# BraveGroup/DCD

Measured on AMD Instinct MI355X. Metric: images/sec DGDE train step (bs=8, 384x1280), higher is better.
Workload: dtype f32; 1 GPU; DGDE train bs=8 fp32 on 1xMI355X, synthetic KITTI 384x1280 + random kpts_ann (DGDE.yaml, DLA-34+DCNv2, 6 objects/image); global_batch=8, per_gpu_batch=8, input=384x1280, parallelism=dp1, dcn_precision=f32, step_launch=eager, sync_bn=False

## Files before the change

### dcd_amd/csrc/dcn_v2.hip

```cpp

#include <hip/hip_runtime.h>
#include <stdint.h>
#include <stdlib.h>
#include <string.h>
#include <atomic>
#include <map>
#include <vector>
#include <mutex>
#include <utility>

#include "../../include/dcd_hip.h"
#include "tuning_env.h"
#include "lds_limit.h"

typedef float f32x16 __attribute__((ext_vector_type(16)));
typedef float f32x32 __attribute__((ext_vector_type(32)));

namespace {

template <int N> struct IntC {
    static constexpr int value = N;
};

struct Geom {
    int B, C, H, W, Co, kh, kw, sh, sw, ph, pw, dh, dw, dg;
    int Ho, Wo, HoWo, KK, cpg, cpgp, Kp, Cop;
};

__host__ inline int round_up(int x, int m) { return (x + m - 1) / m * m; }

__host__ inline bool make_geom(Geom &g, int B, int C, int H, int W, int Co, int kh, int kw, int sh, int sw, int ph,
                               int pw, int dh, int dw, int dg)
{
    if (B <= 0 || C <= 0 || H <= 0 || W <= 0 || Co <= 0 || kh <= 0 || kw <= 0 || sh <= 0 || sw <= 0 || ph < 0 ||
        pw < 0 || dh <= 0 || dw <= 0 || dg <= 0 || C % dg)
        return false;
    g.B = B; g.C = C; g.H = H; g.W = W; g.Co = Co; g.kh = kh; g.kw = kw; g.sh = sh; g.sw = sw;
    g.ph = ph; g.pw = pw; g.dh = dh; g.dw = dw; g.dg = dg;
    g.Ho = (H + 2 * ph - (dh * (kh - 1) + 1)) / sh + 1;
    g.Wo = (W + 2 * pw - (dw * (kw - 1) + 1)) / sw + 1;
    if (g.Ho <= 0 || g.Wo <= 0) return false;
    g.HoWo = g.Ho * g.Wo;
    g.KK = kh * kw;
    g.cpg = C / dg;
    g.cpgp = round_up(g.cpg, 32);
    g.Kp = dg * g.KK * g.cpgp;
    g.Cop = round_up(Co, 32);
    if ((int64_t)C * H * W >= (1ll << 31) || (int64_t)Co * g.HoWo >= (1ll << 31) ||
        (int64_t)g.Kp * g.Cop >= (1ll << 31) || (int64_t)dg * 2 * g.KK * g.HoWo >= (1ll << 31))
        return false;
    return true;
}

__device__ __forceinline__ void prep_weights_body(const float *__restrict__ w, float *__restrict__ wf, float *__restrict__ wb, const Geom &g,
                                                  int bid, int nb)
{
    const int n = g.Kp * g.Cop;
    for (int idx = bid * blockDim.x + threadIdx.x; idx < n; idx += nb * blockDim.x) {
        const int o = idx / g.Kp, kp = idx - o * g.Kp;
        const int seg = kp / g.cpgp, cc = kp - seg * g.cpgp;
        const int grp = seg / g.KK, t = seg - grp * g.KK;
        float v = 0.f;
        if (o < g.Co && cc < g.cpg) v = w[((size_t)o * g.C + grp * g.cpg + cc) * g.KK + t];
        wb[idx] = v;
        wf[(size_t)kp * g.Cop + o] = v;
    }
}
__global__ void dcn_prep_weights(const float *__restrict__ w, float *__restrict__ wf, float *__restrict__ wb, Geom g)
{
    prep_weights_body(w, wf, wb, g, blockIdx.x, gridDim.x);
}

struct Tap {
    int i1, i2, i3, i4;
    float w1, w2, w3, w4;
    float lh, lw, hh, hw;
    float m;
    float oh, ow;
    int pt, pb;
    float a0, a1, b0, b1;
    int shift;
    bool c1, c2, c3, c4;
};

struct TapRaw { float oh, ow, m; };

__device__ __forceinline__ TapRaw load_tap_raw(const float *__restrict__ off_b, const float *__restrict__ msk_b, const Geom &g,
                                               int seg, int Pc)
{
    TapRaw r;
    r.oh = off_b[(size_t)(2 * seg) * g.HoWo + Pc];
    r.ow = off_b[(size_t)(2 * seg + 1) * g.HoWo + Pc];
    r.m = msk_b[(size_t)seg * g.HoWo + Pc];
    return r;
}

__device__ __forceinline__ Tap finish_tap(const TapRaw &raw, const Geom &g, int t, int ho, int wo, bool pv)
{
    Tap s;
    const int i = t / g.kw, j = t - i * g.kw;
    const float oh = raw.oh, ow = raw.ow, m = raw.m;
    const float hf = (float)(ho * g.sh - g.ph + i * g.dh) + oh;
    const float wf = (float)(wo * g.sw - g.pw + j * g.dw) + ow;
    const bool sv = pv && hf > -1.f && wf > -1.f && hf < (float)g.H && wf < (float)g.W;
    const float hlf = sv ? floorf(hf) : 0.f, wlf = sv ? floorf(wf) : 0.f;
    const int hl = (int)hlf, wl = (int)wlf, hh_i = hl + 1, wh_i = wl + 1;
    s.lh = sv ? hf - hlf : 0.f;
    s.lw = sv ? wf - wlf : 0.f;
    s.hh = 1.f - s.lh;
    s.hw = 1.f - s.lw;
    s.c1 = sv && hl >= 0 && wl >= 0;
    s.c2 = sv && hl >= 0 && wh_i <= g.W - 1;
    s.c3 = sv && hh_i <= g.H - 1 && wl >= 0;
    s.c4 = sv && hh_i <= g.H - 1 && wh_i <= g.W - 1;
    s.i1 = s.c1 ? hl * g.W + wl : 0;
    s.i2 = s.c2 ? hl * g.W + wh_i : 0;
    s.i3 = s.c3 ? hh_i * g.W + wl : 0;
    s.i4 = s.c4 ? hh_i * g.W + wh_i : 0;
    s.w1 = s.c1 ? s.hh * s.hw : 0.f;
    s.w2 = s.c2 ? s.hh * s.lw : 0.f;
    s.w3 = s.c3 ? s.lh * s.hw : 0.f;
    s.w4 = s.c4 ? s.lh * s.lw : 0.f;
    s.m = sv ? m : 0.f;
    s.oh = oh;
    s.ow = ow;
    {
        const int xb = g.W >= 2 ? min(max(wl, 0), g.W - 2) : 0;
        const int ya = min(max(hl, 0), g.H - 1), yb = min(max(hh_i, 0), g.H - 1);
        const int shift = xb - wl;
        s.pt = ya * g.W + xb;
        s.pb = yb * g.W + xb;
        s.shift = shift;
        s.a0 = shift == 0 ? s.w1 : (shift == 1 ? s.w2 : 0.f);
        s.a1 = shift == 0 ? s.w2 : (shift == -1 ? s.w1 : 0.f);
        s.b0 = shift == 0 ? s.w3 : (shift == 1 ? s.w4 : 0.f);
        s.b1 = shift == 0 ? s.w4 : (shift == -1 ? s.w3 : 0.f);
        if (!sv) { s.pt = 0; s.pb = 0; }
    }
    return s;
}

__device__ __forceinline__ Tap make_tap(const float *__restrict__ off_b, const float *__restrict__ msk_b, const Geom &g,
                                        int seg, int t, int ho, int wo, int Pc, bool pv)
{
    return finish_tap(load_tap_raw(off_b, msk_b, g, seg, Pc), g, t, ho, wo, pv);
}

__device__ __forceinline__ void xcd_remap(int &bx, int &by)
{
    const int gx = gridDim.x, NT = gx * gridDim.y;
    const int L = bx + gx * by;
    const int xc = L & 7, slot = L >> 3;
    const int q = NT >> 3, r = NT & 7;
    const int Lp = (xc < r ? xc * (q + 1) : r * (q + 1) + (xc - r) * q) + slot;
    by = Lp / gx;
    bx = Lp - by * gx;
}

__device__ __forceinline__ float ldg(const float *base, unsigned byte_off)
{
    return *(const float *)((const char *)base + byte_off);
}

typedef float f32x2 __attribute__((ext_vector_type(2)));
__device__ __forceinline__ f32x2 ldg2(const float *base, unsigned byte_off)
{
    typedef f32x2 __attribute__((aligned(4))) f32x2_u;
    return *(const f32x2_u *)((const char *)base + byte_off);
}

template <int MB>
__global__ __launch_bounds__(256) void dcn_fwd_f32(const float *__restrict__ in, const float *__restrict__ off,
                                                   const float *__restrict__ msk, const float *__restrict__ wf,
                                                   const float *__restrict__ bias, float *__restrict__ out, Geom g)
{
    const int lane = threadIdx.x & 63, wave = threadIdx.x >> 6;
    const int p = lane & 31, h = lane >> 5;
    int bx = blockIdx.x, b = blockIdx.y;
    xcd_remap(bx, b);
    const int tile = bx * 4 + wave;
    if (tile * 32 >= g.HoWo) return;
    const int ob0 = blockIdx.z * MB;
    const int P = tile * 32 + p;
    const bool pv = P < g.HoWo;
    const int Pc = pv ? P : g.HoWo - 1;
    const int ho = Pc / g.Wo, wo = Pc - ho * g.Wo;
    const unsigned HW4 = (unsigned)(g.H * g.W) * 4u;
    const unsigned Cop4 = (unsigned)g.Cop * 4u;

    f32x16 acc[MB];
#pragma unroll
    for (int mb = 0; mb < MB; ++mb)
#pragma unroll
        for (int r = 0; r < 16; ++r) acc[mb][r] = 0.f;

    const float *in_b = in + (size_t)b * g.C * g.H * g.W;
    const float *off_b = off + (size_t)b * g.dg * 2 * g.KK * g.HoWo;
    const float *msk_b = msk + (size_t)b * g.dg * g.KK * g.HoWo;
    const int npair = g.cpg >> 1;
    const unsigned wlane = ((unsigned)h * (unsigned)g.Cop + (unsigned)(ob0 * 32 + p)) * 4u;

    for (int seg = 0; seg < g.dg * g.KK; ++seg) {
        const int grp = seg / g.KK, t = seg - grp * g.KK;
        const Tap s = make_tap(off_b, msk_b, g, seg, t, ho, wo, Pc, pv);
        const float *ip = in_b + (size_t)grp * g.cpg * g.H * g.W;
        const float *wp = wf + (size_t)seg * g.cpgp * g.Cop;
        const unsigned o1 = (unsigned)s.i1 * 4u + h * HW4, o2 = (unsigned)s.i2 * 4u + h * HW4;
        const unsigned o3 = (unsigned)s.i3 * 4u + h * HW4, o4 = (unsigned)s.i4 * 4u + h * HW4;
        const unsigned opt = (unsigned)s.pt * 4u + h * HW4, opb = (unsigned)s.pb * 4u + h * HW4;
        const bool pairs = g.W >= 2;
        const float q1 = pairs ? s.a0 : s.w1, q2 = pairs ? s.a1 : s.w2, q3 = pairs ? s.b0 : s.w3, q4 = pairs ? s.b1 : s.w4;
#ifndef DCN_FWD_UN
#define DCN_FWD_UN ((MB >= 4) ? 2 : 4)
#endif
        constexpr int UN = DCN_FWD_UN;
        float va[UN][4], vb[UN][4], wa[UN][MB], wb_[UN][MB];
        auto issue = [&](float (&v)[UN][4], float (&a)[UN][MB], int it0) {
#pragma unroll
            for (int u = 0; u < UN; ++u) {
                const float *ipc = (const float *)((const char *)ip + (size_t)(it0 + u) * 2 * HW4);
                const float *wpc = (const float *)((const char *)wp + (size_t)(it0 + u) * 2 * Cop4);
#ifdef DCN_ABL_NOGATHER
                v[u][0] = s.w1 + (float)u; v[u][1] = s.w2; v[u][2] = s.w3; v[u][3] = s.w4; (void)ipc;
#else
                if (pairs) {
                    const f32x2 tp = ldg2(ipc, opt), bt = ldg2(ipc, opb);
                    v[u][0] = tp.x; v[u][1] = tp.y; v[u][2] = bt.x; v[u][3] = bt.y;
                } else {
                    v[u][0] = ldg(ipc, o1); v[u][1] = ldg(ipc, o2); v[u][2] = ldg(ipc, o3); v[u][3] = ldg(ipc, o4);
                }
#endif
#pragma unroll
                for (int mb = 0; mb < MB; ++mb)
#ifdef DCN_ABL_NOWEIGHT
                    a[u][mb] = s.w1 + (float)(mb + u); (void)wpc;
#else
                    a[u][mb] = ldg(wpc, wlane + mb * 128u);
#endif
            }
        };
        auto compute = [&](float (&v)[UN][4], float (&a)[UN][MB]) {
#pragma unroll
            for (int u = 0; u < UN; ++u) {
                const float val = (q1 * v[u][0] + q2 * v[u][1] + q3 * v[u][2] + q4 * v[u][3]) * s.m;
#pragma unroll
                for (int mb = 0; mb < MB; ++mb) acc[mb] = __builtin_amdgcn_mfma_f32_32x32x2f32(a[u][mb], val, acc[mb], 0, 0, 0);
            }
        };
        const int nfull = npair / UN;
        int gq = 0;
        if (nfull > 0) issue(va, wa, 0);
        for (; gq + 1 < nfull; gq += 2) {
            issue(vb, wb_, (gq + 1) * UN);
            compute(va, wa);
            if (gq + 2 < nfull) issue(va, wa, (gq + 2) * UN);
            compute(vb, wb_);
        }
        if (gq < nfull) compute(va, wa);
        for (int it = nfull * UN; it < npair; ++it) {
            const float *ipc = (const float *)((const char *)ip + (size_t)it * 2 * HW4);
            const float *wpc = (const float *)((const char *)wp + (size_t)it * 2 * Cop4);
            const float v1 = ldg(ipc, o1), v2 = ldg(ipc, o2), v3 = ldg(ipc, o3), v4 = ldg(ipc, o4);
            const float val = (s.w1 * v1 + s.w2 * v2 + s.w3 * v3 + s.w4 * v4) * s.m;
#pragma unroll
            for (int mb = 0; mb < MB; ++mb)
                acc[mb] = __builtin_amdgcn_mfma_f32_32x32x2f32(ldg(wpc, wlane + mb * 128u), val, acc[mb], 0, 0, 0);
        }
        ip = (const float *)((const char *)ip + (size_t)npair * 2 * HW4);
        wp = (const float *)((const char *)wp + (size_t)npair * 2 * Cop4);
        if (g.cpg & 1) {
            const float v1 = ldg(ip, (unsigned)s.i1 * 4u), v2 = ldg(ip, (unsigned)s.i2 * 4u);
            const float v3 = ldg(ip, (unsigned)s.i3 * 4u), v4 = ldg(ip, (unsigned)s.i4 * 4u);
            float val = (s.w1 * v1 + s.w2 * v2 + s.w3 * v3 + s.w4 * v4) * s.m;
            val = h ? 0.f : val;
#pragma unroll
            for (int mb = 0; mb < MB; ++mb)
                acc[mb] = __builtin_amdgcn_mfma_f32_32x32x2f32(ldg(wp, wlane + mb * 128u), val, acc[mb], 0, 0, 0);
        }
    }

    float *out_b = out + (size_t)b * g.Co * g.HoWo;
#pragma unroll
    for (int mb = 0; mb < MB; ++mb) {
        const int obase = (ob0 + mb) * 32 + 4 * h;
#pragma unroll
        for (int r = 0; r < 16; ++r) {
            const int o = obase + (r & 3) + 8 * (r >> 2);
            if (pv && o < g.Co) out_b[(size_t)o * g.HoWo + P] = acc[mb][r] + bias[o];
        }
    }
}

constexpr int TL_WW = 40;
constexpr int TL_CH = 8;
constexpr int TL_OB = 64;
constexpr int TL_W_FLOATS = 9 * TL_OB * TL_CH;
constexpr int TL_NW = TL_W_FLOATS / 4;
template <int TR> struct TileCfg {
    static constexpr int WH = TR + 8;
    static constexpr int PLANE = (WH * TL_WW) % 64 == 32 ? WH * TL_WW : WH * TL_WW + 32;
    static constexpr int IN_FLOATS = TL_CH * PLANE;
    static constexpr int BUF = IN_FLOATS + TL_W_FLOATS;
    static constexpr int NIN = TL_CH * WH * (TL_WW / 4);
    static constexpr int NT = TR * 64;
    static constexpr int KIN = (NIN + NT - 1) / NT, KW = (TL_NW + NT - 1) / NT;
};


__global__ void dcn_prep_weights9(const float *__restrict__ w, float *__restrict__ wf9, Geom g)
{
    const int K = g.C * 9, n = K * g.Cop;
    for (int idx = blockIdx.x * blockDim.x + threadIdx.x; idx < n; idx += gridDim.x * blockDim.x) {
        const int k = idx / g.Cop, o = idx - k * g.Cop;
        wf9[idx] = (o < g.Co) ? w[(size_t)o * K + k] : 0.f;
    }
}

template <int MB, bool RESCUE = false>
__global__ __launch_bounds__(256) void dcn_fwd9_f32(const float *__restrict__ in, const float *__restrict__ off,
                                                    const float *__restrict__ msk, const float *__restrict__ wf9,
                                                    const float *__restrict__ bias, float *__restrict__ out, Geom g,
                                                    const unsigned char *__restrict__ rescue_flags = nullptr, int tiles_x = 0,
                                                    int rows_per_region = 0, int nchunk = 0)
{
    const int lane = threadIdx.x & 63, wave = threadIdx.x >> 6;
    const int p = lane & 31, h = lane >> 5;
    int bx = blockIdx.x, b = blockIdx.y;
    xcd_remap(bx, b);
    const int tile = bx * 4 + wave;
    const int ob0 = blockIdx.z * MB;
    int P, ho, wo;
    bool pv;
    if (RESCUE) {
        const int row = tile / tiles_x, cseg = tile - row * tiles_x;
        if (row >= g.Ho) return;
        const int regions_y = (g.Ho + rows_per_region - 1) / rows_per_region;
        if (!rescue_flags[((size_t)b * regions_y + row / rows_per_region) * tiles_x + cseg]) return;
        ho = row;
        wo = cseg * 32 + p;
        pv = wo < g.Wo;
        if (!pv) wo = g.Wo - 1;
        P = ho * g.Wo + wo;
    } else {
        if (tile * 32 >= g.HoWo) return;
        P = tile * 32 + p;
        pv = P < g.HoWo;
        if (!pv) P = g.HoWo - 1;
        ho = P / g.Wo;
        wo = P - ho * g.Wo;
    }
    const int Pc = P;
    const unsigned HW4 = (unsigned)(g.H * g.W) * 4u;
    const unsigned Cop4 = (unsigned)g.Cop * 4u;

    f32x16 acc[MB];
#pragma unroll
    for (int mb = 0; mb < MB; ++mb)
#pragma unroll
        for (int r = 0; r < 16; ++r) acc[mb][r] = 0.f;

    const float *in_b = in + (size_t)b * g.C * g.H * g.W;
    const float *off_b = off + (size_t)b * g.dg * 18 * g.HoWo;
    const float *msk_b = msk + (size_t)b * g.dg * 9 * g.HoWo;
    const unsigned wlane = (unsigned)(ob0 * 32 + p) * 4u;
    const int npair = g.cpg >> 1;

    for (int grp = 0; grp < g.dg; ++grp) {
        unsigned to[9][2];
        float tw[9][4];
#pragma unroll
        for (int t = 0; t < 9; ++t) {
            const Tap s = make_tap(off_b, msk_b, g, grp * 9 + t, t, ho, wo, Pc, pv);
            to[t][0] = (unsigned)s.pt * 4u; to[t][1] = (unsigned)s.pb * 4u;
            tw[t][0] = s.a0 * s.m; tw[t][1] = s.a1 * s.m; tw[t][2] = s.b0 * s.m; tw[t][3] = s.b1 * s.m;
        }
        const float *ip = in_b + ((size_t)grp * g.cpg + h) * g.H * g.W;
        const float *wp = wf9 + ((size_t)grp * g.cpg + h) * 9 * g.Cop;
        auto pair_step = [&](const float *ipc, const float *wpc, bool live) {
#pragma unroll
            for (int t0 = 0; t0 < 9; t0 += 3) {
                f32x2 vt[3], vb[3];
                float a[3][MB];
#pragma unroll
                for (int u = 0; u < 3; ++u) {
                    vt[u] = ldg2(ipc, to[t0 + u][0]);
                    vb[u] = ldg2(ipc, to[t0 + u][1]);
#pragma unroll
                    for (int mb = 0; mb < MB; ++mb) a[u][mb] = ldg(wpc, wlane + (unsigned)(t0 + u) * Cop4 + mb * 128u);
                }
#pragma unroll
                for (int u = 0; u < 3; ++u) {
                    float val = tw[t0 + u][0] * vt[u].x + tw[t0 + u][1] * vt[u].y + tw[t0 + u][2] * vb[u].x + tw[t0 + u][3] * vb[u].y;
                    val = live ? val : 0.f;
#pragma unroll
                    for (int mb = 0; mb < MB; ++mb)
                        acc[mb] = __builtin_amdgcn_mfma_f32_32x32x2f32(a[u][mb], val, acc[mb], 0, 0, 0);
                }
            }
        };
        for (int it = 0; it < npair; ++it)
            pair_step((const float *)((const char *)ip + (size_t)it * 2 * HW4),
                      (const float *)((const char *)wp + (size_t)it * 18 * Cop4), true);
        if (g.cpg & 1) {
            const size_t back = h ? (size_t)g.H * g.W : 0;
            const size_t wback = h ? (size_t)9 * g.Cop : 0;
            pair_step((const float *)((const char *)ip + (size_t)npair * 2 * HW4) - back,
                      (const float *)((const char *)wp + (size_t)npair * 18 * Cop4) - wback, h == 0);
        }
    }

    float *out_b = out + (size_t)b * g.Co * g.HoWo;
#pragma unroll
    for (int mb = 0; mb < MB; ++mb) {
        const int obase = (ob0 + mb) * 32 + 4 * h;
#pragma unroll
        for (int r = 0; r < 16; ++r) {
            const int o = obase + (r & 3) + 8 * (r >> 2);
            if (pv && o < g.Co) out_b[(size_t)o * g.HoWo + Pc] = acc[mb][r] + bias[o];
        }
    }
}

typedef float f32x4 __attribute__((ext_vector_type(4)));

__global__ void dcn_prep_weights_tile(const float *__restrict__ w, float *__restrict__ wl, Geom g, int nchunk, int nz,
                                      unsigned *__restrict__ flags, int nflag_words, float *__restrict__ wf9)
{
    for (int i = blockIdx.x * blockDim.x + threadIdx.x; i < nflag_words; i += gridDim.x * blockDim.x) flags[i] = 0u;
    if (wf9) {
        const int K = g.C * 9, n9 = K * g.Cop;
        for (int idx = blockIdx.x * blockDim.x + threadIdx.x; idx < n9; idx += gridDim.x * blockDim.x) {
            const int k = idx / g.Cop, o = idx - k * g.Cop;
            wf9[idx] = (o < g.Co) ? w[(size_t)o * K + k] : 0.f;
        }
    }
    const int n = nz * nchunk * TL_W_FLOATS;
    for (int idx = blockIdx.x * blockDim.x + threadIdx.x; idx < n; idx += gridDim.x * blockDim.x) {
        int r = idx;
        const int s = r & 3; r >>= 2;
        const int h = r & 1; r >>= 1;
        const int o = r % TL_OB; r /= TL_OB;
        const int t = r % 9; r /= 9;
        const int ck = r % nchunk, z = r / nchunk;
        const int oo = z * TL_OB + o, c = ck * TL_CH + 2 * s + h;
        wl[idx] = (oo < g.Co && c < g.C) ? w[((size_t)oo * g.C + c) * 9 + t] : 0.f;
    }
}

constexpr float TL_NEAR_F = 3.f;
__global__ __launch_bounds__(256) void dcn_fwd_far_count(const float *__restrict__ off, int64_t n, unsigned *__restrict__ counter)
{
    unsigned c = 0;
    const int64_t n4 = ((uintptr_t)off & 15) == 0 ? n >> 2 : 0;
    for (int64_t i = (int64_t)blockIdx.x * blockDim.x + threadIdx.x; i < n4; i += (int64_t)gridDim.x * blockDim.x) {
        const f32x4 v = *reinterpret_cast<const f32x4 *>(off + 4 * i);
        c += (!(fabsf(v.x) < TL_NEAR_F)) + (!(fabsf(v.y) < TL_NEAR_F)) + (!(fabsf(v.z) < TL_NEAR_F)) + (!(fabsf(v.w) < TL_NEAR_F));
    }
    for (int64_t i = 4 * n4 + (int64_t)blockIdx.x * blockDim.x + threadIdx.x; i < n; i += (int64_t)gridDim.x * blockDim.x)
        c += !(fabsf(off[i]) < TL_NEAR_F);
#pragma unroll
    for (int o = 32; o > 0; o >>= 1) c += __shfl_xor(c, o);
    __shared__ unsigned part[4];
    if ((threadIdx.x & 63) == 0) part[threadIdx.x >> 6] = c;
    __syncthreads();
    if (threadIdx.x == 0 && part[0] + part[1] + part[2] + part[3]) atomicAdd(counter, part[0] + part[1] + part[2] + part[3]);
}

template <int TR>
__global__ __launch_bounds__(TR * 64) void dcn_fwd_tile_f32(const float *__restrict__ in, const float *__restrict__ off,
                                                        const float *__restrict__ msk, const float *__restrict__ wl,
                                                        const float *__restrict__ bias, float *__restrict__ out, Geom g,
                                                        int tiles_x, int nchunk, unsigned char *__restrict__ rescue_flags,
                                                        const float *__restrict__ wf9, int rescue_taps,
                                                        const unsigned *__restrict__ far_count, unsigned far_limit)
{
    typedef TileCfg<TR> T;
    constexpr int TL_ROWS = TR, TL_WH = T::WH, TL_PLANE = T::PLANE, TL_IN_FLOATS = T::IN_FLOATS, TL_BUF = T::BUF,
                  TL_NIN = T::NIN, NT = T::NT, KIN = T::KIN, KW = T::KW;
    extern __shared__ __attribute__((aligned(16))) float lds[];
    const int tid = threadIdx.x;
    const int lane = tid & 63, wave = tid >> 6;
    const int p = lane & 31, h = lane >> 5;
    int bx = blockIdx.x, b = blockIdx.y;
    xcd_remap(bx, b);
    if (*far_count > far_limit) {
        if (tid == 0) rescue_flags[(size_t)b * gridDim.x + bx] = 1;
        return;
    }
    const int ty = bx / tiles_x, tx = bx - ty * tiles_x;
    const int r0 = ty * TL_ROWS, c0 = tx * 32;
    const int ho = r0 + wave, wo = c0 + p;
    const bool pv = ho < g.Ho && wo < g.Wo;
    const int Pc = pv ? ho * g.Wo + wo : 0;
    const int z = blockIdx.z;
    const int HW = g.H * g.W;
    const int Y0 = r0 - 4, X0 = c0 - 4;

    const float *in_b = in + (size_t)b * g.C * HW;
    const float *off_b = off + (size_t)b * 18 * g.HoWo;
    const float *msk_b = msk + (size_t)b * 9 * g.HoWo;
    const float *wl_z = wl + (size_t)z * nchunk * TL_W_FLOATS;

    int sg[KIN], sl[KIN];
    bool sv_[KIN];
#pragma unroll
    for (int k = 0; k < KIN; ++k) {
        const int e = tid + NT * k;
        const int ch = e / (TL_WH * 10), rem = e - ch * (TL_WH * 10);
        const int row = rem / 10, q = rem - row * 10;
        const int y = Y0 + row, x = X0 + 4 * q;
        sv_[k] = e < TL_NIN;
        sg[k] = (sv_[k] && y >= 0 && y < g.H && x >= 0 && x < g.W) ? ch * HW + y * g.W + x : -1;
        sl[k] = ch * TL_PLANE + row * TL_WW + 4 * q;
    }
    f32x4 rin[KIN];
    auto issue_w = [&](int ck, float *buf) {
        const float *src = wl_z + (size_t)ck * TL_W_FLOATS + 4 * tid;
        float *dst = buf + TL_IN_FLOATS + 4 * 64 * __builtin_amdgcn_readfirstlane(wave);
#pragma unroll
        for (int k = 0; k < KW; ++k)
            if (64 * __builtin_amdgcn_readfirstlane(wave) + NT * k < TL_NW)
                __builtin_amdgcn_global_load_lds(src + 4 * NT * k, (__attribute__((address_space(3))) void *)(dst + 4 * NT * k), 16, 0, 0);
    };
    auto issue = [&](int ck) {
        const float *src = in_b + (size_t)ck * TL_CH * HW;
        const int cleft = g.C - ck * TL_CH;
#pragma unroll
        for (int k = 0; k < KIN; ++k) {
            const f32x4 zero4 = {0.f, 0.f, 0.f, 0.f};
            rin[k] = zero4;
            if (sv_[k] && sg[k] >= 0 && (tid + NT * k) / (TL_WH * 10) < cleft) rin[k] = *reinterpret_cast<const f32x4 *>(src + sg[k]);
        }
    };
    auto commit = [&](float *buf) {
#pragma unroll
        for (int k = 0; k < KIN; ++k)
            if (sv_[k]) *reinterpret_cast<f32x4 *>(buf + sl[k]) = rin[k];
    };

    issue(0);

    int lo[9];
    float wq[9][4];
    unsigned farbits = 0;
#pragma unroll
    for (int t = 0; t < 9; ++t) {
        const TapRaw raw = load_tap_raw(off_b, msk_b, g, t, Pc);
        const float hf = (float)(ho - 1 + t / 3) + raw.oh, wf_ = (float)(wo - 1 + t % 3) + raw.ow;
        const bool sv = pv && hf > -1.f && wf_ > -1.f && hf < (float)g.H && wf_ < (float)g.W;
        const float hlf = floorf(hf), wlf = floorf(wf_);
        const int ly = sv ? (int)hlf - Y0 : 0, lx = sv ? (int)wlf - X0 : 0;
        const bool inside = ly >= 0 && lx >= 0 && ly <= TL_WH - 2 && lx <= TL_WW - 2;
        farbits |= (sv && !inside) ? (1u << t) : 0u;
        lo[t] = (inside ? ly * TL_WW + lx : 0) + h * TL_PLANE;
        const float lh = hf - hlf, lw = wf_ - wlf;
        const float m = (sv && inside) ? raw.m : 0.f;
        wq[t][0] = (1.f - lh) * (1.f - lw) * m; wq[t][1] = (1.f - lh) * lw * m;
        wq[t][2] = lh * (1.f - lw) * m;         wq[t][3] = lh * lw * m;
    }

    f32x16 acc[2];
#pragma unroll
    for (int mb = 0; mb < 2; ++mb)
#pragma unroll
        for (int r = 0; r < 16; ++r) acc[mb][r] = 0.f;

    int wave_far_taps = 0;
#pragma unroll
    for (int t = 0; t < 9; ++t) wave_far_taps += __any((farbits >> t) & 1u) ? 1 : 0;
    __shared__ int far_worst;
    if (tid == 0) far_worst = 0;
    __syncthreads();
    if (lane == 0) atomicMax(&far_worst, wave_far_taps);
    __syncthreads();
    if (far_worst >= rescue_taps) {
        if (tid == 0) rescue_flags[(size_t)b * gridDim.x + bx] = 1;
        return;
    }

    issue_w(0, lds);
    commit(lds);
    asm volatile("s_waitcnt vmcnt(0)" ::: "memory");
    __syncthreads();

    for (int ck = 0; ck < nchunk; ++ck) {
        const float *buf = lds + (ck & 1) * TL_BUF;
#ifndef TL_ABL_NOSTAGE
        if (ck + 1 < nchunk) {
            issue_w(ck + 1, lds + ((ck + 1) & 1) * TL_BUF);
            issue(ck + 1);
        }
#endif
        const float *wb_ = buf + TL_IN_FLOATS + (p * 2 + h) * 4;
#pragma unroll
        for (int t = 0; t < 9; ++t) {
#ifdef TL_ABL_NOW
            const f32x4 a0 = {wq[t][0], wq[t][1], wq[t][2], wq[t][3]}, a1 = {wq[t][1], wq[t][0], wq[t][3], wq[t][2]};
            (void)wb_;
#else
            const f32x4 a0 = *reinterpret_cast<const f32x4 *>(wb_ + (t * TL_OB) * 8);
            const f32x4 a1 = *reinterpret_cast<const f32x4 *>(wb_ + (t * TL_OB + 32) * 8);
#endif
            const float *cp = buf + lo[t];
            const float q0 = wq[t][0], q1 = wq[t][1], q2 = wq[t][2], q3 = wq[t][3];
#pragma unroll
            for (int s = 0; s < 4; ++s) {
                const float *c2 = cp + 2 * s * TL_PLANE;
#ifdef TL_ABL_NOLDS
                const float val = q0 * (float)s + q1 + q2 * (float)ck + q3;
                (void)c2;
#else
                const float val = q0 * c2[0] + q1 * c2[1] + q2 * c2[TL_WW] + q3 * c2[TL_WW + 1];
#endif
                acc[0] = __builtin_amdgcn_mfma_f32_32x32x2f32(a0[s], val, acc[0], 0, 0, 0);
                acc[1] = __builtin_amdgcn_mfma_f32_32x32x2f32(a1[s], val, acc[1], 0, 0, 0);
            }
        }
#ifndef TL_ABL_NOSTAGE
        if (ck + 1 < nchunk) commit(lds + ((ck + 1) & 1) * TL_BUF);
#endif
        asm volatile("s_waitcnt vmcnt(0)" ::: "memory");
#ifndef TL_ABL_NOBAR
        __syncthreads();
#endif
    }

    if (__any(farbits != 0u)) {
#pragma unroll 1
        for (int t = 0; t < 9; ++t) {
            if (!__any((farbits >> t) & 1u)) continue;
            const bool mine = (farbits >> t) & 1u;
            const Tap s = make_tap(off_b, msk_b, g, t, t, ho, wo, Pc, pv);
            const float *w9 = wf9 + (size_t)t * g.Cop + z * TL_OB + p;
            const bool second = z * TL_OB + 32 < g.Cop;
            const int cend = (g.C + 1) & ~1;
            for (int c0 = h; c0 < cend; c0 += 8) {
                f32x2 gt[4], gb[4];
                float wa[4], wb2[4];
#pragma unroll
                for (int u = 0; u < 4; ++u) {
                    const int c = c0 + 2 * u;
                    const int cc = c < g.C ? c : g.C - 1;
                    const float *gp = in_b + (size_t)cc * HW;
                    gt[u] = ldg2(gp, (unsigned)s.pt * 4u);
                    gb[u] = ldg2(gp, (unsigned)s.pb * 4u);
                    const float *wr = w9 + (size_t)cc * 9 * g.Cop;
                    wa[u] = wr[0];
                    wb2[u] = second ? wr[32] : 0.f;
                }
#pragma unroll
                for (int u = 0; u < 4; ++u) {
                    const int c = c0 + 2 * u;
                    const bool live = mine && c < g.C;
                    const float val = live ? (s.a0 * gt[u].x + s.a1 * gt[u].y + s.b0 * gb[u].x + s.b1 * gb[u].y) * s.m : 0.f;
                    acc[0] = __builtin_amdgcn_mfma_f32_32x32x2f32(wa[u], val, acc[0], 0, 0, 0);
                    acc[1] = __builtin_amdgcn_mfma_f32_32x32x2f32(wb2[u], val, acc[1], 0, 0, 0);
                }
            }
        }
    }

    float *out_b = out + (size_t)b * g.Co * g.HoWo;
#pragma unroll
    for (int mb = 0; mb < 2; ++mb) {
        const int obase = z * TL_OB + mb * 32 + 4 * h;
#pragma unroll
        for (int r = 0; r < 16; ++r) {
            const int o = obase + (r & 3) + 8 * (r >> 2);
            if (pv && o < g.Co) out_b[(size_t)o * g.HoWo + ho * g.Wo + wo] = acc[mb][r] + bias[o];
        }
    }
}

constexpr float TL_NEAR = 3.f;
constexpr unsigned FAR_BY_COUNT = 0x80000000u;
constexpr unsigned FAR_COUNT_PIVOT = 0x40000000u;
__device__ __forceinline__ bool far_dominated(const unsigned *far_scal, int total_tiles)
{
    if (!far_scal) return false;
    const unsigned c = far_scal[3];
    if (c & FAR_BY_COUNT) return (c & ~FAR_BY_COUNT) > FAR_COUNT_PIVOT;
    return (int64_t)far_scal[1] * 2 > (int64_t)total_tiles;
}

inline unsigned far_count_limit(const Geom &g, bool wide)
{
    static const int div = dcd_env("DCD_FAR_DIV") ? atoi(dcd_env("DCD_FAR_DIV")) : 0;
    static const int div_wide = dcd_env("DCD_FAR_DIV_WIDE") ? atoi(dcd_env("DCD_FAR_DIV_WIDE")) : 0;
    int d = wide ? div_wide : div;
    if (d <= 0) d = wide ? (g.B >= 4 ? 16 : 8) : (g.B >= 4 ? 24 : 12);
    const int64_t total = (int64_t)g.B * 18 * g.HoWo;
    int64_t lim = total / d;
    if (lim > (int64_t)FAR_COUNT_PIVOT - 1) lim = FAR_COUNT_PIVOT - 1;
    return (unsigned)lim;
}

struct HandoverState {
    unsigned *host = nullptr;
    unsigned *dev = nullptr;
};
static std::mutex g_handover_mu;
static std::map<std::pair<int, const void *>, HandoverState> g_handover;
static std::map<int, std::vector<HandoverState>> g_handover_free;
constexpr unsigned HANDOVER_UNKNOWN = 0xffffffffu;

static std::atomic<int> g_handover_pin{-1};
static int handover_mode()
{
    const int pin = g_handover_pin.load(std::memory_order_relaxed);
    if (pin >= 0) return pin;
    static const int m = [] {
        const char *e = dcd_env("DCD_DCN_HANDOVER");
        if (e && !strcmp(e, "always")) return 1;
        if (e && !strcmp(e, "never")) return 0;
        return 2;
    }();
    return m;
}

static bool stream_is_capturing(hipStream_t stream)
{
    hipStreamCaptureStatus st = hipStreamCaptureStatusNone;
    return hipStreamIsCapturing(stream, &st) == hipSuccess && st != hipStreamCaptureStatusNone;
}

static int handover_decide(hipStream_t stream, const void *weight, unsigned real_limit, unsigned **report)
{
    *report = nullptr;
    const int mode = handover_mode();
    if (mode != 2) return mode;
    int dev = 0;
    (void)hipGetDevice(&dev);
    std::lock_guard<std::mutex> lock(g_handover_mu);
    HandoverState &h = g_handover[std::make_pair(dev, weight)];
    if (!h.host) {
        std::vector<HandoverState> &fl = g_handover_free[dev];
        if (!fl.empty()) {
            h = fl.back();
            fl.pop_back();
            *report = h.dev;
            return 1;
        }
        if (stream_is_capturing(stream)) return 1;
        unsigned *hp = nullptr, *dp = nullptr;
        if (hipHostMalloc((void **)&hp, sizeof(unsigned), hipHostMallocMapped) != hipSuccess ||
            hipHostGetDevicePointer((void **)&dp, hp, 0) != hipSuccess) {
            (void)hipGetLastError();
            if (hp) (void)hipHostFree(hp);
            return 1;
        }
        *hp = HANDOVER_UNKNOWN;
        h.host = hp;
        h.dev = dp;
    }
    *report = h.dev;
    const unsigned far = *(volatile unsigned *)h.host;
    return (far == HANDOVER_UNKNOWN || (uint64_t)far * 2 > real_limit) ? 1 : 0;
}

static bool handover_far_dominated(const void *weight, unsigned real_limit, unsigned **report)
{
    *report = nullptr;
    if (handover_mode() != 2) return false;
    int dev = 0;
    (void)hipGetDevice(&dev);
    std::lock_guard<std::mutex> lock(g_handover_mu);
    auto it = g_handover.find(std::make_pair(dev, weight));
    if (it == g_handover.end() || !it->second.host) return false;
    const unsigned far = *(volatile unsigned *)it->second.host;
    if (far == HANDOVER_UNKNOWN || far <= real_limit) return false;
    *report = it->second.dev;
    return true;
}

__global__ void dcn_far_report(const unsigned *__restrict__ scal, unsigned *__restrict__ report)
{
    if (threadIdx.x == 0 && blockIdx.x == 0) *report = scal[3] & ~FAR_BY_COUNT;
}

static bool forward_keeps_far_samples(const void *weight, int64_t ncoord)
{
    const int mode = handover_mode();
    if (mode != 2) return mode == 0;
    int dev = 0;
    (void)hipGetDevice(&dev);
    std::lock_guard<std::mutex> lock(g_handover_mu);
    auto it = g_handover.find(std::make_pair(dev, weight));
    if (it == g_handover.end() || !it->second.host) return false;
    const unsigned far = *(volatile unsigned *)it->second.host;
    return far != HANDOVER_UNKNOWN && (int64_t)far * 64 <= ncoord;
}

constexpr int INV_CAP = 10;
constexpr int INV_RCAP = 8;
constexpr int INV_RTILE = 3;
constexpr int INV_OVERFLOW = 255;

struct InvLists {
    const unsigned *absmax_bits;
    unsigned char *cnt;
    int *idx;
    float *w;
    int packed;
    const unsigned char *blockmax;
    unsigned char *tileflag;
    int flag_tx, flag_ty;
};

__device__ __forceinline__ int inv_radius(const unsigned *absmax_bits)
{
    const float m = __uint_as_float(*absmax_bits);
    int r = (m == m) ? (int)ceilf(fminf(m, 1e6f)) : INV_RCAP;
    return r > INV_RCAP ? INV_RCAP : r;
}

__device__ __forceinline__ void offset_absmax_body(const float *__restrict__ off, int64_t n, unsigned *__restrict__ scal, int HoWo,
                                                   int ch_per_img, int tiles_per_img, unsigned char *__restrict__ far_flag,
                                                   int *__restrict__ far_list, int bid, int nb)
{
    float m = 0.f;
    unsigned nfar = 0u;
    auto visit = [&](int64_t i, float raw) {
        const float v = fabsf(raw);
        m = fmaxf(m, v);
        if (!(v < TL_NEAR)) {
            ++nfar;
            if (!far_flag) return;
            const int64_t plane = i / HoWo;
            const int P = (int)(i - plane * HoWo), b = (int)(plane / ch_per_img);
            const int tid_ = b * tiles_per_img + (P >> 5);
            if (__builtin_nontemporal_load(far_flag + tid_) == 0) {
                unsigned *word = (unsigned *)(far_flag + (tid_ & ~3));
                const unsigned bit = 1u << (8 * (tid_ & 3));
                if ((atomicOr(word, bit) & bit) == 0u) far_list[atomicAdd(scal + 1, 1u)] = tid_;
            }
        }
    };
    const int64_t n4 = ((uintptr_t)off & 15) == 0 ? n >> 2 : 0;
    for (int64_t i = (int64_t)bid * blockDim.x + threadIdx.x; i < n4; i += (int64_t)nb * blockDim.x) {
        const f32x4 v = *reinterpret_cast<const f32x4 *>(off + 4 * i);
        visit(4 * i, v.x); visit(4 * i + 1, v.y); visit(4 * i + 2, v.z); visit(4 * i + 3, v.w);
    }
    for (int64_t i = 4 * n4 + (int64_t)bid * blockDim.x + threadIdx.x; i < n; i += (int64_t)nb * blockDim.x)
        visit(i, off[i]);
#pragma unroll
    for (int o = 32; o > 0; o >>= 1) { m = fmaxf(m, __shfl_xor(m, o)); nfar += __shfl_xor(nfar, o); }
    __shared__ float part[4];
    __shared__ unsigned partn[4];
    if ((threadIdx.x & 63) == 0) { part[threadIdx.x >> 6] = m; partn[threadIdx.x >> 6] = nfar; }
    __syncthreads();
    if (threadIdx.x == 0) {
        atomicMax(scal, __float_as_uint(fmaxf(fmaxf(part[0], part[1]), fmaxf(part[2], part[3]))));
        const unsigned nf = partn[0] + partn[1] + partn[2] + partn[3];
        if (nf) atomicAdd(scal + 3, nf);
    }
}
__global__ void dcn_offset_absmax(const float *__restrict__ off, int64_t n, unsigned *__restrict__ scal, int HoWo,
                                  int ch_per_img, int tiles_per_img, unsigned char *__restrict__ far_flag,
                                  int *__restrict__ far_list)
{
    offset_absmax_body(off, n, scal, HoWo, ch_per_img, tiles_per_img, far_flag, far_list, blockIdx.x, gridDim.x);
}

__global__ __launch_bounds__(64) void dcn_offset_blockmax(const float *__restrict__ off, Geom g, unsigned char *__restrict__ blockmax,
                                                          const unsigned *__restrict__ only_if_far = nullptr)
{
    if (only_if_far && !far_dominated(only_if_far, g.B * ((g.HoWo + 31) / 32))) return;
    const int nbx = (g.Wo + 7) >> 3, nby = (g.Ho + 7) >> 3;
    const int blk = blockIdx.x, seg = blockIdx.y, b = blockIdx.z;
    const int by = blk / nbx, bx = blk - by * nbx;
    const int S = g.dg * g.KK;
    const int py = by * 8 + (threadIdx.x >> 3), px = bx * 8 + (threadIdx.x & 7);
    float m = 0.f;
    if (py < g.Ho && px < g.Wo) {
        const float *oh_p = off + ((size_t)b * S + seg) * 2 * g.HoWo;
        const int P = py * g.Wo + px;
        m = fmaxf(fabsf(oh_p[P]), fabsf(oh_p[g.HoWo + P]));
        if (!(m == m)) m = 1e6f;
    }
#pragma unroll
    for (int o = 32; o > 0; o >>= 1) m = fmaxf(m, __shfl_xor(m, o));
    if (threadIdx.x == 0) blockmax[(((size_t)b * S + seg) * nby + by) * nbx + bx] = (unsigned char)fminf(ceilf(m), 255.f);
}

__global__ __launch_bounds__(256) void dcn_build_inverse(const float *__restrict__ off, const float *__restrict__ msk,
                                                         InvLists inv, Geom g, const unsigned *__restrict__ only_if_far = nullptr)
{
    if (only_if_far && !far_dominated(only_if_far, g.B * ((g.HoWo + 31) / 32))) return;
    const int HW = g.H * g.W;
    const int q = blockIdx.x * 256 + threadIdx.x;
    if (q >= HW) return;
    const int seg = blockIdx.y, b = blockIdx.z;
    const int S = g.dg * g.KK;
    const int t = seg % g.KK, i = t / g.kw, j = t - i * g.kw;
    const int qy = q / g.W, qx = q - qy * g.W;
    const int rg = inv_radius(inv.absmax_bits);
    const int cy = qy + g.ph - i * g.dh, cx = qx + g.pw - j * g.dw;
    int rm1 = rg;
    if (inv.blockmax) {
        const int nbx = (g.Wo + 7) >> 3, nby = (g.Ho + 7) >> 3;
        const int pcy = min(max(cy / g.sh, 0), g.Ho - 1) >> 3, pcx = min(max(cx / g.sw, 0), g.Wo - 1) >> 3;
        const unsigned char *bm = inv.blockmax + ((size_t)b * S + seg) * nby * nbx;
        int r0 = 0;
        for (int dy = -1; dy <= 1; ++dy)
            for (int dx = -1; dx <= 1; ++dx) {
                const int yy = pcy + dy, xx = pcx + dx;
                if (yy >= 0 && yy < nby && xx >= 0 && xx < nbx) r0 = max(r0, (int)bm[yy * nbx + xx]);
            }
        if (r0 <= 7 && r0 < rg) rm1 = r0;
    }
    if (inv.tileflag && rm1 > INV_RTILE) inv.tileflag[((size_t)b * inv.flag_ty + (qy >> 2)) * inv.flag_tx + (qx >> 5)] = 1;
    const int R = rm1 + 1;
    const float rlim = (float)rg;
    const float *oh_p = off + ((size_t)b * S + seg) * 2 * g.HoWo;
    const float *ow_p = oh_p + g.HoWo;
    const float *m_p = msk + ((size_t)b * S + seg) * g.HoWo;
    const size_t base = ((size_t)b * S + seg) * INV_CAP * HW + q;
    int py0 = (cy - R + g.sh - 1) / g.sh, py1 = (cy + R) / g.sh;
    int px0 = (cx - R + g.sw - 1) / g.sw, px1 = (cx + R) / g.sw;
// ... 1850 lines not shown
```

Measured before the change: 216.0 images/s.

## Interleave channel pairs in LDS tile and software-pipeline tap reads in DCN forward

Changes the shared-memory input tile layout so that pairs of channels are interleaved per pixel. Each bilinear corner read becomes a single 2-float load serving two channels instead of separate scalar loads from different planes, and the tile weight packing is reordered to match. The inner tap loop is also software-pipelined: the next tap's weights and corner values are prefetched before the MFMA calls, with a sched_barrier fixing the order. This cuts the number of LDS reads and hides their latency behind matrix ops, at the cost of more registers and dropping the bank-conflict padding that the old plane stride had.

New measurement: 215.1 images/s. Within noise of the previous version (-0.4%).

```diff
diff --git a/dcd_amd/csrc/dcn_v2.hip b/dcd_amd/csrc/dcn_v2.hip
--- a/dcd_amd/csrc/dcn_v2.hip
+++ b/dcd_amd/csrc/dcn_v2.hip
@@ -298,10 +298,11 @@
 constexpr int TL_NW = TL_W_FLOATS / 4;
 template <int TR> struct TileCfg {
     static constexpr int WH = TR + 8;
-    static constexpr int PLANE = (WH * TL_WW) % 64 == 32 ? WH * TL_WW : WH * TL_WW + 32;
-    static constexpr int IN_FLOATS = TL_CH * PLANE;
+    static constexpr int GRP = 2 * TL_WW;
+    static constexpr int ROW = 4 * GRP;
+    static constexpr int IN_FLOATS = WH * ROW;
     static constexpr int BUF = IN_FLOATS + TL_W_FLOATS;
-    static constexpr int NIN = TL_CH * WH * (TL_WW / 4);
+    static constexpr int NIN = 4 * WH * (TL_WW / 4);
     static constexpr int NT = TR * 64;
     static constexpr int KIN = (NIN + NT - 1) / NT, KW = (TL_NW + NT - 1) / NT;
 };
@@ -438,11 +439,12 @@
     for (int idx = blockIdx.x * blockDim.x + threadIdx.x; idx < n; idx += gridDim.x * blockDim.x) {
         int r = idx;
         const int s = r & 3; r >>= 2;
+        const int o = r & 31; r >>= 5;
         const int h = r & 1; r >>= 1;
-        const int o = r % TL_OB; r /= TL_OB;
+        const int mb = r & 1; r >>= 1;
         const int t = r % 9; r /= 9;
         const int ck = r % nchunk, z = r / nchunk;
-        const int oo = z * TL_OB + o, c = ck * TL_CH + 2 * s + h;
+        const int oo = z * TL_OB + mb * 32 + o, c = ck * TL_CH + 2 * s + h;
         wl[idx] = (oo < g.Co && c < g.C) ? w[((size_t)oo * g.C + c) * 9 + t] : 0.f;
     }
 }
@@ -475,7 +477,7 @@
                                                         const unsigned *__restrict__ far_count, unsigned far_limit)
 {
     typedef TileCfg<TR> T;
-    constexpr int TL_ROWS = TR, TL_WH = T::WH, TL_PLANE = T::PLANE, TL_IN_FLOATS = T::IN_FLOATS, TL_BUF = T::BUF,
+    constexpr int TL_ROWS = TR, TL_WH = T::WH, TL_ROW = T::ROW, TL_GRP = T::GRP, TL_IN_FLOATS = T::IN_FLOATS, TL_BUF = T::BUF,
                   TL_NIN = T::NIN, NT = T::NT, KIN = T::KIN, KW = T::KW;
     extern __shared__ __attribute__((aligned(16))) float lds[];
     const int tid = threadIdx.x;
@@ -501,19 +503,20 @@
     const float *msk_b = msk + (size_t)b * 9 * g.HoWo;
     const float *wl_z = wl + (size_t)z * nchunk * TL_W_FLOATS;
 
-    int sg[KIN], sl[KIN];
+    int sg[KIN], sl[KIN], sca[KIN];
     bool sv_[KIN];
 #pragma unroll
     for (int k = 0; k < KIN; ++k) {
         const int e = tid + NT * k;
-        const int ch = e / (TL_WH * 10), rem = e - ch * (TL_WH * 10);
+        const int gq = e / (TL_WH * 10), rem = e - gq * (TL_WH * 10);
         const int row = rem / 10, q = rem - row * 10;
         const int y = Y0 + row, x = X0 + 4 * q;
         sv_[k] = e < TL_NIN;
-        sg[k] = (sv_[k] && y >= 0 && y < g.H && x >= 0 && x < g.W) ? ch * HW + y * g.W + x : -1;
-        sl[k] = ch * TL_PLANE + row * TL_WW + 4 * q;
-    }
-    f32x4 rin[KIN];
+        sca[k] = 4 * (gq >> 1) + (gq & 1);
+        sg[k] = (sv_[k] && y >= 0 && y < g.H && x >= 0 && x < g.W) ? sca[k] * HW + y * g.W + x : -1;
+        sl[k] = row * TL_ROW + gq * TL_GRP + 8 * q;
+    }
+    f32x4 rin[KIN][2];
     auto issue_w = [&](int ck, float *buf) {
         const float *src = wl_z + (size_t)ck * TL_W_FLOATS + 4 * tid;
         float *dst = buf + TL_IN_FLOATS + 4 * 64 * __builtin_amdgcn_readfirstlane(wave);
@@ -528,14 +531,19 @@
 #pragma unroll
         for (int k = 0; k < KIN; ++k) {
             const f32x4 zero4 = {0.f, 0.f, 0.f, 0.f};
-            rin[k] = zero4;
-            if (sv_[k] && sg[k] >= 0 && (tid + NT * k) / (TL_WH * 10) < cleft) rin[k] = *reinterpret_cast<const f32x4 *>(src + sg[k]);
+            rin[k][0] = zero4; rin[k][1] = zero4;
+            if (sv_[k] && sg[k] >= 0 && sca[k] < cleft) rin[k][0] = *reinterpret_cast<const f32x4 *>(src + sg[k]);
+            if (sv_[k] && sg[k] >= 0 && sca[k] + 2 < cleft) rin[k][1] = *reinterpret_cast<const f32x4 *>(src + sg[k] + 2 * HW);
         }
     };
     auto commit = [&](float *buf) {
 #pragma unroll
         for (int k = 0; k < KIN; ++k)
-            if (sv_[k]) *reinterpret_cast<f32x4 *>(buf + sl[k]) = rin[k];
+            if (sv_[k]) {
+                const f32x4 a = rin[k][0], b2 = rin[k][1];
+                *reinterpret_cast<f32x4 *>(buf + sl[k]) = f32x4{a.x, b2.x, a.y, b2.y};
+                *reinterpret_cast<f32x4 *>(buf + sl[k] + 4) = f32x4{a.z, b2.z, a.w, b2.w};
+            }
     };
 
     issue(0);
@@ -552,7 +560,7 @@
         const int ly = sv ? (int)hlf - Y0 : 0, lx = sv ? (int)wlf - X0 : 0;
         const bool inside = ly >= 0 && lx >= 0 && ly <= TL_WH - 2 && lx <= TL_WW - 2;
         farbits |= (sv && !inside) ? (1u << t) : 0u;
-        lo[t] = (inside ? ly * TL_WW + lx : 0) + h * TL_PLANE;
+        lo[t] = (inside ? ly * TL_ROW + 2 * lx : 0) + h * TL_GRP;
         const float lh = hf - hlf, lw = wf_ - wlf;
         const float m = (sv && inside) ? raw.m : 0.f;
         wq[t][0] = (1.f - lh) * (1.f - lw) * m; wq[t][1] = (1.f - lh) * lw * m;
@@ -591,30 +599,49 @@
             issue(ck + 1);
         }
 #endif
-        const float *wb_ = buf + TL_IN_FLOATS + (p * 2 + h) * 4;
-#pragma unroll
-        for (int t = 0; t < 9; ++t) {
+        const float *wb_ = buf + TL_IN_FLOATS + (h * 32 + p) * 4;
+        auto read_w = [&](int t, f32x4 &a0, f32x4 &a1) {
 #ifdef TL_ABL_NOW
-            const f32x4 a0 = {wq[t][0], wq[t][1], wq[t][2], wq[t][3]}, a1 = {wq[t][1], wq[t][0], wq[t][3], wq[t][2]};
+            a0 = f32x4{wq[t][0], wq[t][1], wq[t][2], wq[t][3]}; a1 = f32x4{wq[t][1], wq[t][0], wq[t][3], wq[t][2]};
             (void)wb_;
 #else
-            const f32x4 a0 = *reinterpret_cast<const f32x4 *>(wb_ + (t * TL_OB) * 8);
-            const f32x4 a1 = *reinterpret_cast<const f32x4 *>(wb_ + (t * TL_OB + 32) * 8);
-#endif
-            const float *cp = buf + lo[t];
+            a0 = *reinterpret_cast<const f32x4 *>(wb_ + (t * TL_OB) * 8);
+            a1 = *reinterpret_cast<const f32x4 *>(wb_ + (t * TL_OB + 32) * 8);
+#endif
+        };
+        auto read_c = [&](int t, int sp, f32x2 (&c)[4]) {
+#ifdef TL_ABL_NOLDS
+            c[0] = f32x2{(float)(2 * sp), (float)(2 * sp + 1)}; c[1] = f32x2{1.f, 1.f};
+            c[2] = f32x2{(float)ck, (float)ck};                 c[3] = f32x2{1.f, 1.f};
+#else
+            const f32x2 *c2 = reinterpret_cast<const f32x2 *>(buf + lo[t] + 2 * sp * TL_GRP);
+            c[0] = c2[0];          c[1] = c2[1];
+            c[2] = c2[TL_ROW / 2]; c[3] = c2[TL_ROW / 2 + 1];
+#endif
+        };
+        f32x4 a0, a1, a0n, a1n;
+        f32x2 c[4], cn[4];
+        read_w(0, a0, a1);
+        read_c(0, 0, c);
+#pragma unroll
+        for (int t = 0; t < 9; ++t) {
             const float q0 = wq[t][0], q1 = wq[t][1], q2 = wq[t][2], q3 = wq[t][3];
 #pragma unroll
-            for (int s = 0; s < 4; ++s) {
-                const float *c2 = cp + 2 * s * TL_PLANE;
-#ifdef TL_ABL_NOLDS
-                const float val = q0 * (float)s + q1 + q2 * (float)ck + q3;
-                (void)c2;
-#else
-                const float val = q0 * c2[0] + q1 * c2[1] + q2 * c2[TL_WW] + q3 * c2[TL_WW + 1];
-#endif
-                acc[0] = __builtin_amdgcn_mfma_f32_32x32x2f32(a0[s], val, acc[0], 0, 0, 0);
-                acc[1] = __builtin_amdgcn_mfma_f32_32x32x2f32(a1[s], val, acc[1], 0, 0, 0);
-            }
+            for (int sp = 0; sp < 2; ++sp) {
+                const float va = q0 * c[0].x + q1 * c[1].x + q2 * c[2].x + q3 * c[3].x;
+                const float vb = q0 * c[0].y + q1 * c[1].y + q2 * c[2].y + q3 * c[3].y;
+                if (sp == 0 && t + 1 < 9) read_w(t + 1, a0n, a1n);
+                if (sp == 0) read_c(t, 1, cn);
+                else if (t + 1 < 9) read_c(t + 1, 0, cn);
+                __builtin_amdgcn_sched_barrier(0);
+                acc[0] = __builtin_amdgcn_mfma_f32_32x32x2f32(a0[2 * sp], va, acc[0], 0, 0, 0);
+                acc[1] = __builtin_amdgcn_mfma_f32_32x32x2f32(a1[2 * sp], va, acc[1], 0, 0, 0);
+                acc[0] = __builtin_amdgcn_mfma_f32_32x32x2f32(a0[2 * sp + 1], vb, acc[0], 0, 0, 0);
+                acc[1] = __builtin_amdgcn_mfma_f32_32x32x2f32(a1[2 * sp + 1], vb, acc[1], 0, 0, 0);
+#pragma unroll
+                for (int i = 0; i < 4; ++i) c[i] = cn[i];
+            }
+            a0 = a0n; a1 = a1n;
         }
 #ifndef TL_ABL_NOSTAGE
         if (ck + 1 < nchunk) commit(lds + ((ck + 1) & 1) * TL_BUF);
```
